# marc345/Dense2Sparse-ViT

Hardware: AMD Instinct MI355X
Metric: training images/s, DeiT-S 224 keep_ratio=0.5 (dense-to-sparse ViT train step, teacher fwd + student fwd/bwd + AdamW) (higher is better)
Workload: dtype f32; 1 GPU; DeiT-Small 224x224 patch16, 1-stage prune keep_ratio=0.5 @ block 3 (196->98 tokens), large LN predictor, kl_div mask loss, per-GPU batch 128; global_batch=128, parallelism=dp1

## Files before the change

dense2sparse-vit_amd/csrc/attention_f32.hip:

```cpp
#include "d2s_common.h"

namespace {

#ifdef D2S_ATTN_STAMPS
__device__ unsigned long long g_attn_stamps[16 * 8192];
#define ASTAMP(i) if (threadIdx.x == 0) { const int L_ = blockIdx.y * gridDim.x + blockIdx.x; if (L_ < 8192) g_attn_stamps[16 * L_ + (i)] = __builtin_amdgcn_s_memtime(); }
#define ASTAMPR(i) if (threadIdx.x == 0) { const int L_ = blockIdx.y * gridDim.x + blockIdx.x; if (L_ < 8192) g_attn_stamps[16 * L_ + (i)] = __builtin_amdgcn_s_memrealtime(); }
#else
#define ASTAMP(i)
#define ASTAMPR(i)
#endif

constexpr int DH = 64;
constexpr int PITCH = 68;

__device__ __forceinline__ void load_rows_regs(const float* __restrict__ base, long ld, int row, int nrows, int half,
                                               float scale, f32x4 (&r)[8]) {
    if (row < nrows) {
        const float* p = base + (long)row * ld + 4 * half;
#pragma unroll
        for (int t = 0; t < 8; ++t) {
            r[t] = *reinterpret_cast<const f32x4*>(p + 8 * t);
#pragma unroll
            for (int j = 0; j < 4; ++j) r[t][j] *= scale;
        }
    } else {
#pragma unroll
        for (int t = 0; t < 8; ++t) r[t] = f32x4{0.f, 0.f, 0.f, 0.f};
    }
}

__device__ __forceinline__ void tile_load(const float* __restrict__ base, long ld, int row0, int nrows, int tid, f32x4 (&r)[2]) {
#pragma unroll
    for (int i = 0; i < 2; ++i) {
        const int f = tid + i * 256, row = row0 + (f >> 4), d4 = (f & 15) * 4;
        r[i] = row < nrows ? *reinterpret_cast<const f32x4*>(base + (long)row * ld + d4) : f32x4{0.f, 0.f, 0.f, 0.f};
    }
}
__device__ __forceinline__ void tile_store(float* __restrict__ S, int tid, const f32x4 (&r)[2]) {
#pragma unroll
    for (int i = 0; i < 2; ++i) {
        const int f = tid + i * 256;
        *reinterpret_cast<f32x4*>(&S[(f >> 4) * PITCH + (f & 15) * 4]) = r[i];
    }
}

__device__ __forceinline__ void mma_lds_reg(const float* __restrict__ S, int l31, int half, const f32x4 (&y)[8], f32x16& acc) {
#pragma unroll
    for (int t = 0; t < 8; ++t) {
        const f32x4 a = *reinterpret_cast<const f32x4*>(&S[l31 * PITCH + 8 * t + 4 * half]);
#pragma unroll
        for (int j = 0; j < 4; ++j) acc = mfma32(a[j], y[t][j], acc);
    }
}
__device__ __forceinline__ void mma_reg_lds(const f32x16& p, const float* __restrict__ S, int l31, int half, f32x16 (&o)[2],
                                            int groups = 4) {
#pragma unroll
    for (int g = 0; g < 4; ++g) {
        if (g < groups) {
#pragma unroll
            for (int r = 4 * g; r < 4 * g + 4; ++r) {
                const float* row = &S[mfma32_row(r, half) * PITCH];
                o[0] = mfma32(p[r], row[l31], o[0]);
                o[1] = mfma32(p[r], row[32 + l31], o[1]);
            }
        }
    }
}

__device__ __forceinline__ void mma_lds_reg_t(const f32x16& p, const float* __restrict__ S, int l31, int half, f32x16 (&o)[2],
                                              int groups = 4) {
#pragma unroll
    for (int g = 0; g < 4; ++g) {
        if (g < groups) {
#pragma unroll
            for (int r = 4 * g; r < 4 * g + 4; ++r) {
                const float* row = &S[mfma32_row(r, half) * PITCH];
                o[0] = mfma32(row[l31], p[r], o[0]);
                o[1] = mfma32(row[32 + l31], p[r], o[1]);
            }
        }
    }
}

struct AttnFwdArgs {
    const float* qkv; float* out; float* lse; float* cls_row;
    const float* policy; float* cinv; const int* cu;
    int n, H; float scale, eps; int total;
};

template <bool POLICY, bool VARLEN, bool KEYW = false>
__global__ __launch_bounds__(256, 3) void attn_fwd_kernel(AttnFwdArgs a) {
    __shared__ __attribute__((aligned(16))) float Ks[32 * PITCH];
    __shared__ __attribute__((aligned(16))) float Vs[32 * PITCH];
    __shared__ float pol_s[32];
    __shared__ __attribute__((aligned(16))) float vred[POLICY ? 16 * 64 : 4];
    __shared__ float vsum_s[64];
    extern __shared__ __attribute__((aligned(16))) float cls_s[];
    const int tid = threadIdx.x, lane = tid & 63, wave = tid >> 6, half = lane >> 5, l31 = lane & 31;
    const int H = a.H;
    ASTAMP(0); ASTAMPR(8);
    int bx, by;
    xcd_remap_2d(bx, by);
    const int b = by / H, h = by % H;
    const long ld = 3L * H * DH;
    const int row_base = VARLEN ? a.cu[b] : 0;
    const int n = VARLEN ? a.cu[b + 1] - row_base : a.n;
    if (VARLEN && bx * 128 >= n) return;
    const long tok0 = VARLEN ? (long)row_base : (long)b * n;
    const float* qb = a.qkv + tok0 * ld + h * DH;
    const float* kb = qb + (long)H * DH;
    const float* vb = kb + (long)H * DH;
    const float* polb = (POLICY || KEYW) ? a.policy + (long)b * n : nullptr;
    const float scale = a.scale;
    const int q0 = bx * 128 + wave * 32;
    const bool active = q0 < n;
    const bool want_cls = a.cls_row != nullptr && bx == 0 && wave == 0;
    const int qi = q0 + l31;

    f32x4 qreg[8];
    load_rows_regs(qb, ld, qi, n, half, scale, qreg);

    f32x16 o[2];
#pragma unroll
    for (int r = 0; r < 16; ++r) { o[0][r] = 0.f; o[1][r] = 0.f; }
    float m_run = -INFINITY, l_run = 0.f;
    f32x4 vacc = {0.f, 0.f, 0.f, 0.f};

    const int ntiles = (n + 31) / 32;
    f32x4 kr[2], vr[2];
    float pr = 0.f;
    tile_load(kb, ld, 0, n, tid, kr);
    tile_load(vb, ld, 0, n, tid, vr);
    if ((POLICY || KEYW) && tid < 32) pr = tid < n ? polb[tid] : 0.f;
    for (int t = 0; t < ntiles; ++t) {
        __syncthreads();
        tile_store(Ks, tid, kr);
        tile_store(Vs, tid, vr);
        if (KEYW && tid < 32) pol_s[tid] = pr;
        if (POLICY) {
            if (tid < 32) pol_s[tid] = pr;
            vacc += vr[0];
            vacc += vr[1];
        }
        __syncthreads();
        if (t == 0) { ASTAMP(1); }
        if (t == 1) { ASTAMP(2); }
        if (t == 2) { ASTAMP(3); }
        if (t + 1 < ntiles) {
            tile_load(kb, ld, (t + 1) * 32, n, tid, kr);
            tile_load(vb, ld, (t + 1) * 32, n, tid, vr);
            if ((POLICY || KEYW) && tid < 32) { const int kj = (t + 1) * 32 + tid; pr = kj < n ? polb[kj] : 0.f; }
        }
        if (!active) continue;
        f32x16 s;
#pragma unroll
        for (int r = 0; r < 16; ++r) s[r] = 0.f;
        mma_lds_reg(Ks, l31, half, qreg, s);
        const int kv0 = t * 32;
        float mt = -INFINITY;
#pragma unroll
        for (int r = 0; r < 16; ++r) {
            if (kv0 + mfma32_row(r, half) >= n) s[r] = -INFINITY;
            mt = fmaxf(mt, s[r]);
        }
        if (want_cls && l31 == 0) {
#pragma unroll
            for (int r = 0; r < 16; ++r) {
                const int key = kv0 + mfma32_row(r, half);
                if (key < n) cls_s[key] = s[r];
            }
        }
        mt = fmaxf(mt, __shfl_xor(mt, 32, 64));
        const float m_new = fmaxf(m_run, mt);
        const float alpha = __expf(m_run - m_new);
        float rs = 0.f;
#pragma unroll
        for (int r = 0; r < 16; ++r) {
            s[r] = __expf(s[r] - m_new);
            if (POLICY) {
                const int kr_ = mfma32_row(r, half);
                s[r] *= (kv0 + kr_ == qi) ? 1.f : pol_s[kr_];
            }
            if (KEYW) s[r] *= pol_s[mfma32_row(r, half)];
            rs += s[r];
        }
        rs += __shfl_xor(rs, 32, 64);
        l_run = l_run * alpha + rs;
        m_run = m_new;
#pragma unroll
        for (int r = 0; r < 16; ++r) {
            o[0][r] *= alpha;
            o[1][r] *= alpha;
        }
        mma_lds_reg_t(s, Vs, l31, half, o, min(4, (n - kv0 + 7) >> 3));
    }
    ASTAMP(4);
    const float c = POLICY ? a.eps / (float)n : 0.f;
    if (POLICY) {
        *reinterpret_cast<f32x4*>(&vred[(tid >> 4) * 64 + (tid & 15) * 4]) = vacc;
        __syncthreads();
        if (tid < 64) {
            float t = 0.f;
#pragma unroll
            for (int g = 0; g < 16; ++g) t += vred[g * 64 + tid];
            vsum_s[tid] = t * c;
        }
        __syncthreads();
    }
    if (!active) return;
    const float inv_l = 1.0f / (POLICY ? l_run + a.eps : l_run);
    if (qi < n) {
        float* p = a.out + (tok0 + qi) * H * DH + h * DH;
#pragma unroll
        for (int dt = 0; dt < 2; ++dt)
#pragma unroll
            for (int g = 0; g < 4; ++g) {
                f32x4 v;
#pragma unroll
                for (int j = 0; j < 4; ++j) {
                    float num = o[dt][4 * g + j];
                    if (POLICY) num += vsum_s[32 * dt + 8 * g + 4 * half + j];
                    v[j] = num * inv_l;
                }
                *reinterpret_cast<f32x4*>(p + 32 * dt + 8 * g + 4 * half) = v;
            }
    }
    const long stat0 = VARLEN ? (long)h * a.total + row_base : ((long)b * H + h) * n;
    if (half == 0 && qi < n) {
        if (a.lse) a.lse[stat0 + qi] = m_run + logf(POLICY ? l_run + a.eps : l_run);
        if (POLICY && a.cinv) a.cinv[stat0 + qi] = c * inv_l;
    }
    if (want_cls) {
        const float m0 = __shfl(m_run, 0, 64), il0 = __shfl(inv_l, 0, 64);
        float* cr = a.cls_row + stat0;
        for (int j = lane; j < n; j += 64) {
            float e = expf(cls_s[j] - m0);
            if (POLICY) e = e * (j == 0 ? 1.f : polb[j]) + c;
            cr[j] = e * il0;
        }
    }
    ASTAMP(5); ASTAMPR(9);
}

__global__ __launch_bounds__(256) void attn_delta_kernel(const float* __restrict__ out, const float* __restrict__ dout,
                                                         float* __restrict__ delta, long rows, int n, int H) {
    const int lane = threadIdx.x & 63;
    const long row = (long)blockIdx.x * 4 + (threadIdx.x >> 6);
    if (row >= rows) return;
    const long b = row / n, i = row - b * n;
    for (int h = 0; h < H; ++h) {
        const long e = row * H * DH + h * DH + lane;
        const float s = wave_sum(out[e] * dout[e]);
        if (lane == 0) delta[(b * H + h) * n + i] = s;
    }
}

__device__ __forceinline__ void tile_load_u32(const float* __restrict__ base, unsigned ld, int row0, int nrows, int tid, f32x4 (&r)[2]) {
#pragma unroll
    for (int i = 0; i < 2; ++i) {
        const int f = tid + i * 256, row = row0 + (f >> 4);
        const unsigned off = (unsigned)row * ld + (unsigned)((f & 15) * 4);
        r[i] = row < nrows ? *reinterpret_cast<const f32x4*>(base + off) : f32x4{0.f, 0.f, 0.f, 0.f};
    }
}

struct VarlenSeg { const int* cu; int total; };
__device__ __forceinline__ int varlen_rows(VarlenSeg v, int b, int max_n, int& row_base) {
    const int r0 = min(max(v.cu[b], 0), v.total), r1 = min(max(v.cu[b + 1], r0), v.total);
    row_base = r0;
    return min(r1 - r0, max_n);
}

template <bool POLICY, bool KEYW = false, bool VARLEN = false>
__global__ __launch_bounds__(256, 3) void attn_bwd_dq_kernel(const float* __restrict__ qkv, const float* __restrict__ dout,
                                                          const float* __restrict__ lse, const float* __restrict__ delta,
                                                          float* __restrict__ dqkv, int n, int H, float scale,
                                                          const float* __restrict__ policy, VarlenSeg varlen) {
    static_assert(!(KEYW && POLICY), "key weights travel in the policy's argument");
    static_assert(!(VARLEN && (POLICY || KEYW)), "the ragged form has neither a policy nor key weights");
    __shared__ __attribute__((aligned(16))) float Ks[32 * PITCH];
    __shared__ __attribute__((aligned(16))) float Vs[32 * PITCH];
    __shared__ float pol_s[32];
    const int tid = threadIdx.x, lane = tid & 63, wave = tid >> 6, half = lane >> 5, l31 = lane & 31;
    int bx, by;
    xcd_remap_2d(bx, by);
    const int b = by / H, h = by % H;
    const long ld = 3L * H * DH, ldo = (long)H * DH;
    int row_base = 0;
    if constexpr (VARLEN) {
        n = varlen_rows(varlen, b, n, row_base);
        if (bx * 128 >= n) return;
    }
    const long stat0v = VARLEN ? (long)h * varlen.total + row_base : 0;
    const float* qb = qkv + (VARLEN ? (long)row_base : (long)b * n) * ld + h * DH;
    const float* kb = qb + (long)H * DH;
    const float* vb = kb + (long)H * DH;
    const float* dob = dout + (VARLEN ? (long)row_base : (long)b * n) * ldo + h * DH;
    const int q0 = bx * 128 + wave * 32;
    const bool active = q0 < n;

    f32x4 qreg[8], doreg[8];
    load_rows_regs(qb, ld, q0 + l31, n, half, scale, qreg);
    load_rows_regs(dob, ldo, q0 + l31, n, half, 1.0f, doreg);
    const bool qok = q0 + l31 < n;
    const float lse_i = qok ? lse[(VARLEN ? stat0v : ((long)b * H + h) * n) + q0 + l31] : INFINITY;
    const float dl_i = qok ? delta[(VARLEN ? stat0v : ((long)b * H + h) * n) + q0 + l31] : 0.f;

    f32x16 dq[2];
#pragma unroll
    for (int r = 0; r < 16; ++r) { dq[0][r] = 0.f; dq[1][r] = 0.f; }

    const int ntiles = (n + 31) / 32;
    f32x4 kr[2], vr[2];
    float pr = 0.f;
    const float* polb = (POLICY || KEYW) ? policy + (long)b * n : nullptr;
    if (VARLEN) {
        tile_load_u32(kb, (unsigned)ld, 0, n, tid, kr);
        tile_load_u32(vb, (unsigned)ld, 0, n, tid, vr);
    } else {
        tile_load(kb, ld, 0, n, tid, kr);
        tile_load(vb, ld, 0, n, tid, vr);
    }
    if ((POLICY || KEYW) && tid < 32) pr = tid < n ? polb[tid] : 0.f;
    for (int t = 0; t < ntiles; ++t) {
        __syncthreads();
        tile_store(Ks, tid, kr);
        tile_store(Vs, tid, vr);
        if ((POLICY || KEYW) && tid < 32) pol_s[tid] = pr;
        __syncthreads();
        if (t + 1 < ntiles) {
            if (VARLEN) {
                tile_load_u32(kb, (unsigned)ld, (t + 1) * 32, n, tid, kr);
                tile_load_u32(vb, (unsigned)ld, (t + 1) * 32, n, tid, vr);
            } else {
                tile_load(kb, ld, (t + 1) * 32, n, tid, kr);
                tile_load(vb, ld, (t + 1) * 32, n, tid, vr);
            }
            if ((POLICY || KEYW) && tid < 32) { const int kj = (t + 1) * 32 + tid; pr = kj < n ? polb[kj] : 0.f; }
        }
        if (!active) continue;
        f32x16 s, dp;
#pragma unroll
        for (int r = 0; r < 16; ++r) { s[r] = 0.f; dp[r] = 0.f; }
        mma_lds_reg(Ks, l31, half, qreg, s);
        mma_lds_reg(Vs, l31, half, doreg, dp);
        const int kv0 = t * 32;
#pragma unroll
        for (int r = 0; r < 16; ++r) {
            const int kr_ = mfma32_row(r, half);
            float p = (kv0 + kr_ < n) ? __expf(s[r] - lse_i) : 0.f;
            if (POLICY) p *= (kv0 + kr_ == q0 + l31) ? 1.f : pol_s[kr_];
            if (KEYW) p *= pol_s[kr_];
            s[r] = p * (dp[r] - dl_i);
        }
        mma_reg_lds(s, Ks, l31, half, dq, min(4, (n - kv0 + 7) >> 3));
    }
    if (!active) return;
    float* dqb = dqkv + (VARLEN ? (long)row_base : (long)b * n) * ld + h * DH;
#pragma unroll
    for (int r = 0; r < 16; ++r) {
        const int qi = q0 + mfma32_row(r, half);
        if (qi < n) {
            float* p = dqb + (long)qi * ld;
            p[l31] = dq[0][r] * scale;
            p[32 + l31] = dq[1][r] * scale;
        }
    }
}

__device__ __forceinline__ void dkv_fetch_next(const float* __restrict__ qb, const float* __restrict__ dob, const float* __restrict__ lse_b,
                                               const float* __restrict__ dl_b, const float* __restrict__ ci_b, unsigned ld, unsigned ldo,
                                               int t1, int n, int tid, f32x4 (&qr)[2], f32x4 (&dr)[2], float& lr, float& dlr, float& cir) {
    tile_load_u32(qb, ld, t1 * 32, n, tid, qr);
    tile_load_u32(dob, ldo, t1 * 32, n, tid, dr);
    if (tid < 32) {
        const unsigned qi = (unsigned)(t1 * 32 + tid);
        lr = qi < (unsigned)n ? lse_b[qi] : INFINITY;
        dlr = qi < (unsigned)n ? dl_b[qi] : 0.f;
        cir = qi < (unsigned)n ? ci_b[qi] : 0.f;
    }
}

template <bool POLICY, bool DPOL = false, bool KEYW = false, bool VARLEN = false>
__global__ __launch_bounds__(256, 2) void attn_bwd_dkv_kernel(const float* __restrict__ qkv, const float* __restrict__ dout,
                                                           const float* __restrict__ lse, const float* __restrict__ delta,
                                                           float* __restrict__ dqkv, int n, int H, float scale,
                                                           const float* __restrict__ policy, const float* __restrict__ cinv,
                                                           float* dpol_part, VarlenSeg varlen) {
    static_assert(!DPOL || POLICY, "the policy's gradient needs a policy");
    static_assert(!(KEYW && POLICY), "key weights travel in the policy's argument");
    static_assert(!(VARLEN && (POLICY || DPOL || KEYW)), "the ragged form has neither a policy nor key weights");
    __shared__ __attribute__((aligned(16))) float Qs[32 * PITCH];
    __shared__ __attribute__((aligned(16))) float Ds[32 * PITCH];
    __shared__ float lse_s[32], dl_s[32], ci_s[32];
    const int tid = threadIdx.x, lane = tid & 63, wave = tid >> 6, half = lane >> 5, l31 = lane & 31;
    int bx, by;
    xcd_remap_2d(bx, by);
    const int b = by / H, h = by % H;
    const long ld = 3L * H * DH, ldo = (long)H * DH;
    int row_base = 0;
    if constexpr (VARLEN) {
        n = varlen_rows(varlen, b, n, row_base);
        if (bx * 128 >= n) return;
    }
    const long tok0 = VARLEN ? (long)row_base : (long)b * n;
    const long stat0 = VARLEN ? (long)h * varlen.total + row_base : ((long)b * H + h) * n;
    const float* qb = qkv + tok0 * ld + h * DH;
    const float* kb = qb + (long)H * DH;
    const float* vb = kb + (long)H * DH;
    const float* dob = dout + tok0 * ldo + h * DH;
    const float* lse_b = lse + stat0;
    const float* dl_b = delta + stat0;
    const int k0 = bx * 128 + wave * 32;
    const bool active = k0 < n;

    f32x4 kreg[8], vreg[8];
    load_rows_regs(kb, ld, k0 + l31, n, half, scale, kreg);
    load_rows_regs(vb, ld, k0 + l31, n, half, 1.0f, vreg);

    f32x16 dk[2], dv[2];
#pragma unroll
    for (int r = 0; r < 16; ++r) { dk[0][r] = 0.f; dk[1][r] = 0.f; dv[0][r] = 0.f; dv[1][r] = 0.f; }

    const int ntiles = (n + 31) / 32;
    f32x4 qr[2], dr[2];
    float lr = 0.f, dlr = 0.f, cir = 0.f;
    float dpol_acc = 0.f;
    const float* ci_b = POLICY ? cinv + ((long)b * H + h) * n : nullptr;
    const float pol_key = ((POLICY || KEYW) && k0 + l31 < n) ? policy[(long)b * n + k0 + l31] : 0.f;
    tile_load(qb, ld, 0, n, tid, qr);
    tile_load(dob, ldo, 0, n, tid, dr);
    if (tid < 32) { lr = tid < n ? lse_b[tid] : INFINITY; dlr = tid < n ? dl_b[tid] : 0.f; if (POLICY) cir = tid < n ? ci_b[tid] : 0.f; }
    for (int t = 0; t < ntiles; ++t) {
        __syncthreads();
        tile_store(Qs, tid, qr);
        tile_store(Ds, tid, dr);
        if (tid < 32) { lse_s[tid] = lr; dl_s[tid] = dlr; if (POLICY) ci_s[tid] = cir; }
        __syncthreads();
        if (!DPOL && t + 1 < ntiles) {
            tile_load(qb, ld, (t + 1) * 32, n, tid, qr);
            tile_load(dob, ldo, (t + 1) * 32, n, tid, dr);
            if (tid < 32) {
                const int qi = (t + 1) * 32 + tid;
                lr = qi < n ? lse_b[qi] : INFINITY;
                dlr = qi < n ? dl_b[qi] : 0.f;
                if (POLICY) cir = qi < n ? ci_b[qi] : 0.f;
            }
        }
        if (DPOL && !active && t + 1 < ntiles) dkv_fetch_next(qb, dob, lse_b, dl_b, ci_b, (unsigned)ld, (unsigned)ldo, t + 1, n, tid, qr, dr, lr, dlr, cir);
        if (!active) continue;
        f32x16 s, dp;
#pragma unroll
        for (int r = 0; r < 16; ++r) { s[r] = 0.f; dp[r] = 0.f; }
        mma_lds_reg(Qs, l31, half, kreg, s);
        mma_lds_reg(Ds, l31, half, vreg, dp);
#pragma unroll
        for (int r = 0; r < 16; ++r) {
            const int qi = mfma32_row(r, half);
            float p = __expf(s[r] - lse_s[qi]);
            if (DPOL) {
                const bool diag = t * 32 + qi == k0 + l31;
                const float g = dp[r] - dl_s[qi];
                dpol_acc += diag ? 0.f : p * g;
                p *= diag ? 1.f : pol_key;
                s[r] = p + ci_s[qi];
                dp[r] = p * g;
                continue;
            }
            if (POLICY) p *= (t * 32 + qi == k0 + l31) ? 1.f : pol_key;
            if (KEYW) p *= pol_key;
            s[r] = POLICY ? p + ci_s[qi] : p;
            dp[r] = p * (dp[r] - dl_s[qi]);
        }
        const int qgroups = min(4, (n - t * 32 + 7) >> 3);
        mma_reg_lds(s, Ds, l31, half, dv, qgroups);
        mma_reg_lds(dp, Qs, l31, half, dk, qgroups);
        if (DPOL && t + 1 < ntiles) dkv_fetch_next(qb, dob, lse_b, dl_b, ci_b, (unsigned)ld, (unsigned)ldo, t + 1, n, tid, qr, dr, lr, dlr, cir);
    }
    if (!active) return;
    int l31e = l31, halfe = half, k0e = k0;
    if constexpr (DPOL) {
        int t2 = (int)threadIdx.x;
        asm volatile("" : "+v"(t2));
        l31e = t2 & 31; halfe = (t2 >> 5) & 1; k0e = bx * 128 + (t2 >> 6) * 32;
        dpol_acc += __shfl_xor(dpol_acc, 32, 64);
        if (halfe == 0 && k0e + l31e < n) dpol_part[((long)b * H + h) * n + k0e + l31e] = dpol_acc;
    }
    float* dkb = dqkv + tok0 * ld + (long)H * DH + h * DH;
    float* dvb = dkb + (long)H * DH;
#pragma unroll
    for (int r = 0; r < 16; ++r) {
        const int ki = k0e + mfma32_row(r, halfe);
        if (ki < n) {
            float* pk = dkb + (long)ki * ld;
            float* pv = dvb + (long)ki * ld;
            pk[l31e] = dk[0][r] * scale;
            pk[32 + l31e] = dk[1][r] * scale;
            pv[l31e] = dv[0][r];
            pv[32 + l31e] = dv[1][r];
        }
    }
}

__global__ __launch_bounds__(256) void attn_dpol_fold_kernel(const float* __restrict__ part, float* __restrict__ dpolicy, int B, int n, int H) {
    const long i = (long)blockIdx.x * 256 + threadIdx.x;
    if (i >= (long)B * n) return;
    const long b = i / n, j = i - b * n;
    float s = 0.f;
    if (j > 0)
        for (int h = 0; h < H; ++h) s += part[(b * H + h) * n + j];
    dpolicy[i] = s;
}

}

#ifdef D2S_ATTN_STAMPS
extern "C" int d2s_debug_read_attn_stamps(unsigned long long* host_out, int n_wg) {
    return hipMemcpyFromSymbol(host_out, HIP_SYMBOL(g_attn_stamps), (size_t)n_wg * 16 * sizeof(unsigned long long)) == hipSuccess ? 0 : -1;
}
#endif

template <bool POLICY, bool VARLEN, bool KEYW = false>
static int attn_fwd_launch(const AttnFwdArgs& a, int B, int n_max, hipStream_t stream) {
    hipLaunchKernelGGL((attn_fwd_kernel<POLICY, VARLEN, KEYW>), dim3((n_max + 127) / 128, B * a.H), dim3(256),
                       a.cls_row ? (size_t)n_max * sizeof(float) : 0, stream, a);
    return d2s_check_launch();
}

template <bool POLICY, bool DPOL = false, bool KEYW = false, bool VARLEN = false>
static int attn_bwd_launch(const float* qkv, const float* out, const float* dout, const float* lse, float* dqkv, float* delta_ws, int B, int n,
                           int H, float scale, hipStream_t stream, const float* policy = nullptr, const float* cinv = nullptr,
                           float* dpolicy = nullptr, float* dpol_ws = nullptr, VarlenSeg seg = VarlenSeg{nullptr, 0}) {
    const long rows = VARLEN ? (long)seg.total : (long)B * n;
    hipLaunchKernelGGL(attn_delta_kernel, dim3((unsigned)((rows + 3) / 4)), dim3(256), 0, stream, out, dout, delta_ws, rows,
                       VARLEN ? seg.total : n, H);
    dim3 grid((n + 127) / 128, B * H), block(256);
    hipLaunchKernelGGL((attn_bwd_dq_kernel<POLICY, KEYW, VARLEN>), grid, block, 0, stream, qkv, dout, lse, delta_ws, dqkv, n, H, scale, policy, seg);
    hipLaunchKernelGGL((attn_bwd_dkv_kernel<POLICY, DPOL, KEYW, VARLEN>), grid, block, 0, stream, qkv, dout, lse, delta_ws, dqkv, n, H, scale,
                       policy, cinv, dpol_ws, seg);
    if (DPOL)
        hipLaunchKernelGGL(attn_dpol_fold_kernel, dim3((unsigned)((rows + 255) / 256)), dim3(256), 0, stream, dpol_ws, dpolicy, B, n, H);
    return d2s_check_launch();
}

static int attn_varlen_fwd(const float* qkv, const int* cu_seqlens, float* out, float* lse, float* cls_row, int B, int total, int max_n, int H,
                           float scale, hipStream_t stream) {
    if (!qkv || !cu_seqlens || !out || B <= 0 || total <= 0 || max_n <= 0 || max_n > 8192 || H <= 0) return D2S_ERR_ARG;
    return attn_fwd_launch<false, true>(AttnFwdArgs{qkv, out, lse, cls_row, nullptr, nullptr, cu_seqlens, 0, H, scale, 0.f, total}, B, max_n, stream);
}

extern "C" {

int d2s_attn_fwd_f32(const float* qkv, float* out, float* lse, float* cls_row, int B, int n, int H, float scale,
                     hipStream_t stream) {
    if (!qkv || !out || !lse || B <= 0 || n <= 0 || H <= 0 || n > 8192) return D2S_ERR_ARG;
    return attn_fwd_launch<false, false>(AttnFwdArgs{qkv, out, lse, cls_row, nullptr, nullptr, nullptr, n, H, scale, 0.f, 0}, B, n, stream);
}

int d2s_attn_policy_fwd_f32(const float* qkv, const float* policy, float* out, float* lse, float* cinv, float* cls_row, int B, int n,
                            int H, float scale, float eps, hipStream_t stream) {
    if (!qkv || !policy || !out || !lse || !cinv || B <= 0 || n <= 0 || H <= 0 || n > 8192) return D2S_ERR_ARG;
    return attn_fwd_launch<true, false>(AttnFwdArgs{qkv, out, lse, cls_row, policy, cinv, nullptr, n, H, scale, eps, 0}, B, n, stream);
}

int d2s_attn_varlen_fwd_f32(const float* qkv, const int* cu_seqlens, float* out, float* cls_row, int B, int total, int max_n, int H,
                            float scale, hipStream_t stream) {
    return attn_varlen_fwd(qkv, cu_seqlens, out, nullptr, cls_row, B, total, max_n, H, scale, stream);
}

int d2s_attn_varlen_fwd_lse_f32(const float* qkv, const int* cu_seqlens, float* out, float* lse, float* cls_row, int B, int total, int max_n,
                                int H, float scale, hipStream_t stream) {
    if (!lse) return D2S_ERR_ARG;
    return attn_varlen_fwd(qkv, cu_seqlens, out, lse, cls_row, B, total, max_n, H, scale, stream);
}

int d2s_attn_varlen_bwd_f32(const float* qkv, const int* cu_seqlens, const float* out, const float* dout, const float* lse, float* dqkv,
                            float* delta_ws, int B, int total, int max_n, int H, float scale, hipStream_t stream) {
    if (!qkv || !cu_seqlens || !out || !dout || !lse || !dqkv || !delta_ws || B <= 0 || total <= 0 || max_n <= 0 || max_n > 8192 || H <= 0)
        return D2S_ERR_ARG;
    if ((long)max_n * 3 * H * 64 >= (1L << 32)) return D2S_ERR_ARG;
    return attn_bwd_launch<false, false, false, true>(qkv, out, dout, lse, dqkv, delta_ws, B, max_n, H, scale, stream, nullptr, nullptr, nullptr,
                                                      nullptr, VarlenSeg{cu_seqlens, total});
}

int d2s_attn_keyw_fwd_f32(const float* qkv, const float* key_w, float* out, float* lse, int B, int n, int H, float scale, hipStream_t stream) {
    if (!qkv || !key_w || !out || B <= 0 || n < 2 || H <= 0 || n > 8192) return D2S_ERR_ARG;
    return attn_fwd_launch<false, false, true>(AttnFwdArgs{qkv, out, lse, nullptr, key_w, nullptr, nullptr, n, H, scale, 0.f, 0}, B, n, stream);
}

int d2s_attn_delta(const float* out, const float* dout, float* delta, int B, int n, int H, hipStream_t stream) {
    if (!out || !dout || !delta || B <= 0 || n <= 0 || H <= 0) return D2S_ERR_ARG;
    const long rows = (long)B * n;
    hipLaunchKernelGGL(attn_delta_kernel, dim3((unsigned)((rows + 3) / 4)), dim3(256), 0, stream, out, dout, delta, rows, n, H);
    return d2s_check_launch();
}

int d2s_attn_bwd_f32(const float* qkv, const float* out, const float* dout, const float* lse, float* dqkv, float* delta_ws, int B,
                     int n, int H, float scale, hipStream_t stream) {
    if (!qkv || !out || !dout || !lse || !dqkv || !delta_ws || B <= 0 || n <= 0 || H <= 0) return D2S_ERR_ARG;
    return attn_bwd_launch<false>(qkv, out, dout, lse, dqkv, delta_ws, B, n, H, scale, stream);
}

int d2s_attn_keyw_bwd_f32(const float* qkv, const float* key_w, const float* out, const float* dout, const float* lse, float* dqkv,
                          float* delta_ws, int B, int n, int H, float scale, hipStream_t stream) {
    if (!qkv || !key_w || !out || !dout || !lse || !dqkv || !delta_ws || B <= 0 || n < 2 || H <= 0 || n > 8192) return D2S_ERR_ARG;
    return attn_bwd_launch<false, false, true>(qkv, out, dout, lse, dqkv, delta_ws, B, n, H, scale, stream, key_w);
}

int d2s_attn_policy_bwd_f32(const float* qkv, const float* policy, const float* out, const float* dout, const float* lse,
                            const float* cinv, float* dqkv, float* delta_ws, int B, int n, int H, float scale, hipStream_t stream) {
    if (!qkv || !policy || !out || !dout || !lse || !cinv || !dqkv || !delta_ws || B <= 0 || n <= 0 || H <= 0) return D2S_ERR_ARG;
    return attn_bwd_launch<true>(qkv, out, dout, lse, dqkv, delta_ws, B, n, H, scale, stream, policy, cinv);
}

int d2s_attn_policy_bwd_dpol_f32(const float* qkv, const float* policy, const float* out, const float* dout, const float* lse,
                                 const float* cinv, float* dqkv, float* delta_ws, float* dpolicy, float* dpol_ws, int B, int n, int H,
                                 float scale, hipStream_t stream) {
    if (!qkv || !policy || !out || !dout || !lse || !cinv || !dqkv || !delta_ws || !dpolicy || !dpol_ws || B <= 0 || n <= 0 || H <= 0)
        return D2S_ERR_ARG;
    if ((long)n * 3 * H * 64 >= (1L << 32)) return D2S_ERR_ARG;
    return attn_bwd_launch<true, true>(qkv, out, dout, lse, dqkv, delta_ws, B, n, H, scale, stream, policy, cinv, dpolicy, dpol_ws);
}

}
```

Baseline: 3616 images/s.

## Handle small remainder key/query tiles with scalar FMA instead of full MFMA tiles

When the sequence length leaves a final tile of at most eight rows (e.g. n=197 or 99 with cls token), the attention forward, dq and dkv kernels now process that last tile with cross-half-wave dot products and scalar FMAs instead of a full 32-row MFMA tile. This is meant to avoid wasting most of an MFMA tile on padding rows. It adds permlane swaps, an LDS transpose buffer for the backward kernels and extra code paths, which may raise register and LDS pressure and affect occupancy.

```diff
diff --git a/dense2sparse-vit_amd/csrc/attention_f32.hip b/dense2sparse-vit_amd/csrc/attention_f32.hip
--- a/dense2sparse-vit_amd/csrc/attention_f32.hip
+++ b/dense2sparse-vit_amd/csrc/attention_f32.hip
@@ -78,6 +78,87 @@
                 const float* row = &S[mfma32_row(r, half) * PITCH];
                 o[0] = mfma32(row[l31], p[r], o[0]);
                 o[1] = mfma32(row[32 + l31], p[r], o[1]);
+            }
+        }
+    }
+}
+
+__device__ __forceinline__ int remainder_rows(int n) { const int rem = n & 31; return rem <= 8 ? rem : 0; }
+__device__ __forceinline__ int remainder_row_at(int i) { return (i >> 1) + 4 * (i & 1); }
+
+__device__ __forceinline__ void half_wave_pair_of(float a, float b, float& x, float& y) {
+    const auto sw = __builtin_amdgcn_permlane32_swap(__float_as_uint(a), __float_as_uint(b), false, false);
+    x = __uint_as_float(sw[0]);
+    y = __uint_as_float(sw[1]);
+}
+__device__ __forceinline__ void dot_rows_lds_reg(const float* __restrict__ S, int half, const f32x4 (&y)[8], int rem, f32x4& s4) {
+    float c[4] = {0.f, 0.f, 0.f, 0.f};
+    const int ni = (rem + 1) >> 1;
+    const float* X = S + half * PITCH;
+#pragma unroll
+    for (int t = 0; t < 8; ++t) {
+        float ylo[4], yhi[4];
+#pragma unroll
+        for (int j = 0; j < 4; ++j) half_wave_pair_of(y[t][j], y[t][j], ylo[j], yhi[j]);
+#pragma unroll
+        for (int i = 0; i < 4; ++i) {
+            if (i < ni) {
+                const f32x4 alo = *reinterpret_cast<const f32x4*>(&X[2 * i * PITCH + 8 * t]);
+                const f32x4 ahi = *reinterpret_cast<const f32x4*>(&X[2 * i * PITCH + 8 * t + 4]);
+#pragma unroll
+                for (int j = 0; j < 4; ++j) {
+                    c[i] = __builtin_fmaf(alo[j], ylo[j], c[i]);
+                    c[i] = __builtin_fmaf(ahi[j], yhi[j], c[i]);
+                }
+            }
+        }
+    }
+    float r0, r1, r2, r3;
+    half_wave_pair_of(c[0], c[2], r0, r1);
+    half_wave_pair_of(c[1], c[3], r2, r3);
+    s4 = f32x4{r0, r1, r2, r3};
+}
+__device__ __forceinline__ float remainder_row_value(const f32x4& p4, int k, int half) {
+    float v = p4[0];
+#pragma unroll
+    for (int r = 1; r < 4; ++r) v = (k & 3) == r ? p4[r] : v;
+    const float other = __shfl_xor(v, 32, 64);
+    return (k >> 2) == half ? v : other;
+}
+__device__ __forceinline__ void fma_lds_reg_t(const f32x4& p4, const float* __restrict__ S, int half, int rem, f32x16 (&o)[2]) {
+#pragma unroll 1
+    for (int i = 0; i < 8; ++i) {
+        const int k = remainder_row_at(i);
+        if (k >= rem) continue;
+        const float pk = remainder_row_value(p4, k, half);
+#pragma unroll
+        for (int dt = 0; dt < 2; ++dt)
+#pragma unroll
+            for (int g = 0; g < 4; ++g) {
+                const f32x4 v = *reinterpret_cast<const f32x4*>(&S[k * PITCH + 32 * dt + 8 * g + 4 * half]);
+#pragma unroll
+                for (int j = 0; j < 4; ++j) o[dt][4 * g + j] = __builtin_fmaf(v[j], pk, o[dt][4 * g + j]);
+            }
+    }
+}
+__device__ __forceinline__ void fma_reg_lds(const f32x4& p4, const float* __restrict__ S, float* T, int l31, int half, int rem,
+                                            f32x16 (&o)[2]) {
+    __builtin_amdgcn_wave_barrier();
+#pragma unroll
+    for (int r = 0; r < 4; ++r) T[(4 * half + r) * 32 + l31] = p4[r];
+    __builtin_amdgcn_wave_barrier();
+#pragma unroll 1
+    for (int i = 0; i < 8; ++i) {
+        const int k = remainder_row_at(i);
+        if (k >= rem) continue;
+        const float s0 = S[k * PITCH + l31], s1 = S[k * PITCH + 32 + l31];
+#pragma unroll
+        for (int g = 0; g < 4; ++g) {
+            const f32x4 w = *reinterpret_cast<const f32x4*>(&T[k * 32 + 8 * g + 4 * half]);
+#pragma unroll
+            for (int j = 0; j < 4; ++j) {
+                o[0][4 * g + j] = __builtin_fmaf(w[j], s0, o[0][4 * g + j]);
+                o[1][4 * g + j] = __builtin_fmaf(w[j], s1, o[1][4 * g + j]);
             }
         }
     }
@@ -128,12 +209,51 @@
     f32x4 vacc = {0.f, 0.f, 0.f, 0.f};
 
     const int ntiles = (n + 31) / 32;
+    const int rem_last = remainder_rows(n), ntiles_mma = ntiles - (rem_last ? 1 : 0);
     f32x4 kr[2], vr[2];
     float pr = 0.f;
     tile_load(kb, ld, 0, n, tid, kr);
     tile_load(vb, ld, 0, n, tid, vr);
     if ((POLICY || KEYW) && tid < 32) pr = tid < n ? polb[tid] : 0.f;
-    for (int t = 0; t < ntiles; ++t) {
+    auto softmax_step = [&](auto& s, int kv0, auto nr) {
+        constexpr int NR = decltype(nr)::value;
+        float mt = -INFINITY;
+#pragma unroll
+        for (int r = 0; r < NR; ++r) {
+            if (kv0 + mfma32_row(r, half) >= n) s[r] = -INFINITY;
+            mt = fmaxf(mt, s[r]);
+        }
+        if (want_cls && l31 == 0) {
+#pragma unroll
+            for (int r = 0; r < NR; ++r) {
+                const int key = kv0 + mfma32_row(r, half);
+                if (key < n) cls_s[key] = s[r];
+            }
+        }
+        mt = fmaxf(mt, __shfl_xor(mt, 32, 64));
+        const float m_new = fmaxf(m_run, mt);
+        const float alpha = __expf(m_run - m_new);
+        float rs = 0.f;
+#pragma unroll
+        for (int r = 0; r < NR; ++r) {
+            s[r] = __expf(s[r] - m_new);
+            if (POLICY) {
+                const int kr_ = mfma32_row(r, half);
+                s[r] *= (kv0 + kr_ == qi) ? 1.f : pol_s[kr_];
+            }
+            if (KEYW) s[r] *= pol_s[mfma32_row(r, half)];
+            rs += s[r];
+        }
+        rs += __shfl_xor(rs, 32, 64);
+        l_run = l_run * alpha + rs;
+        m_run = m_new;
+#pragma unroll
+        for (int r = 0; r < 16; ++r) {
+            o[0][r] *= alpha;
+            o[1][r] *= alpha;
+        }
+    };
+    auto stage_tile = [&]() {
         __syncthreads();
         tile_store(Ks, tid, kr);
         tile_store(Vs, tid, vr);
@@ -144,6 +264,9 @@
             vacc += vr[1];
         }
         __syncthreads();
+    };
+    for (int t = 0; t < ntiles_mma; ++t) {
+        stage_tile();
         if (t == 0) { ASTAMP(1); }
         if (t == 1) { ASTAMP(2); }
         if (t == 2) { ASTAMP(3); }
@@ -153,47 +276,22 @@
             if ((POLICY || KEYW) && tid < 32) { const int kj = (t + 1) * 32 + tid; pr = kj < n ? polb[kj] : 0.f; }
         }
         if (!active) continue;
+        const int kv0 = t * 32;
         f32x16 s;
 #pragma unroll
         for (int r = 0; r < 16; ++r) s[r] = 0.f;
         mma_lds_reg(Ks, l31, half, qreg, s);
-        const int kv0 = t * 32;
-        float mt = -INFINITY;
-#pragma unroll
-        for (int r = 0; r < 16; ++r) {
-            if (kv0 + mfma32_row(r, half) >= n) s[r] = -INFINITY;
-            mt = fmaxf(mt, s[r]);
-        }
-        if (want_cls && l31 == 0) {
-#pragma unroll
-            for (int r = 0; r < 16; ++r) {
-                const int key = kv0 + mfma32_row(r, half);
-                if (key < n) cls_s[key] = s[r];
-            }
-        }
-        mt = fmaxf(mt, __shfl_xor(mt, 32, 64));
-        const float m_new = fmaxf(m_run, mt);
-        const float alpha = __expf(m_run - m_new);
-        float rs = 0.f;
-#pragma unroll
-        for (int r = 0; r < 16; ++r) {
-            s[r] = __expf(s[r] - m_new);
-            if (POLICY) {
-                const int kr_ = mfma32_row(r, half);
-                s[r] *= (kv0 + kr_ == qi) ? 1.f : pol_s[kr_];
-            }
-            if (KEYW) s[r] *= pol_s[mfma32_row(r, half)];
-            rs += s[r];
-        }
-        rs += __shfl_xor(rs, 32, 64);
-        l_run = l_run * alpha + rs;
-        m_run = m_new;
-#pragma unroll
-        for (int r = 0; r < 16; ++r) {
-            o[0][r] *= alpha;
-            o[1][r] *= alpha;
-        }
+        softmax_step(s, kv0, std::integral_constant<int, 16>{});
         mma_lds_reg_t(s, Vs, l31, half, o, min(4, (n - kv0 + 7) >> 3));
+    }
+    if (rem_last) {
+        stage_tile();
+        if (active) {
+            f32x4 s4;
+            dot_rows_lds_reg(Ks, half, qreg, rem_last, s4);
+            softmax_step(s4, (ntiles - 1) * 32, std::integral_constant<int, 4>{});
+            fma_lds_reg_t(s4, Vs, half, rem_last, o);
+        }
     }
     ASTAMP(4);
     const float c = POLICY ? a.eps / (float)n : 0.f;
@@ -282,6 +380,7 @@
     __shared__ __attribute__((aligned(16))) float Ks[32 * PITCH];
     __shared__ __attribute__((aligned(16))) float Vs[32 * PITCH];
     __shared__ float pol_s[32];
+    __shared__ __attribute__((aligned(16))) float tr_s[4 * 8 * 32];
     const int tid = threadIdx.x, lane = tid & 63, wave = tid >> 6, half = lane >> 5, l31 = lane & 31;
     int bx, by;
     xcd_remap_2d(bx, by);
@@ -304,6 +403,7 @@
     load_rows_regs(qb, ld, q0 + l31, n, half, scale, qreg);
     load_rows_regs(dob, ldo, q0 + l31, n, half, 1.0f, doreg);
     const bool qok = q0 + l31 < n;
+    const int wave_u = __builtin_amdgcn_readfirstlane(wave);
     const float lse_i = qok ? lse[(VARLEN ? stat0v : ((long)b * H + h) * n) + q0 + l31] : INFINITY;
     const float dl_i = qok ? delta[(VARLEN ? stat0v : ((long)b * H + h) * n) + q0 + l31] : 0.f;
 
@@ -312,6 +412,7 @@
     for (int r = 0; r < 16; ++r) { dq[0][r] = 0.f; dq[1][r] = 0.f; }
 
     const int ntiles = (n + 31) / 32;
+    const int rem_last = remainder_rows(n), ntiles_mma = ntiles - (rem_last ? 1 : 0);
     f32x4 kr[2], vr[2];
     float pr = 0.f;
     const float* polb = (POLICY || KEYW) ? policy + (long)b * n : nullptr;
@@ -323,12 +424,26 @@
         tile_load(vb, ld, 0, n, tid, vr);
     }
     if ((POLICY || KEYW) && tid < 32) pr = tid < n ? polb[tid] : 0.f;
-    for (int t = 0; t < ntiles; ++t) {
+    auto ds_step = [&](auto& s, const auto& dp, int kv0, int half, auto nr) {
+        constexpr int NR = decltype(nr)::value;
+#pragma unroll
+        for (int r = 0; r < NR; ++r) {
+            const int kr_ = mfma32_row(r, half);
+            float p = (kv0 + kr_ < n) ? __expf(s[r] - lse_i) : 0.f;
+            if (POLICY) p *= (kv0 + kr_ == q0 + l31) ? 1.f : pol_s[kr_];
+            if (KEYW) p *= pol_s[kr_];
+            s[r] = p * (dp[r] - dl_i);
+        }
+    };
+    auto stage_tile = [&]() {
         __syncthreads();
         tile_store(Ks, tid, kr);
         tile_store(Vs, tid, vr);
         if ((POLICY || KEYW) && tid < 32) pol_s[tid] = pr;
         __syncthreads();
+    };
+    for (int t = 0; t < ntiles_mma; ++t) {
+        stage_tile();
         if (t + 1 < ntiles) {
             if (VARLEN) {
                 tile_load_u32(kb, (unsigned)ld, (t + 1) * 32, n, tid, kr);
@@ -340,31 +455,37 @@
             if ((POLICY || KEYW) && tid < 32) { const int kj = (t + 1) * 32 + tid; pr = kj < n ? polb[kj] : 0.f; }
         }
         if (!active) continue;
+        const int kv0 = t * 32;
         f32x16 s, dp;
 #pragma unroll
         for (int r = 0; r < 16; ++r) { s[r] = 0.f; dp[r] = 0.f; }
         mma_lds_reg(Ks, l31, half, qreg, s);
         mma_lds_reg(Vs, l31, half, doreg, dp);
-        const int kv0 = t * 32;
-#pragma unroll
-        for (int r = 0; r < 16; ++r) {
-            const int kr_ = mfma32_row(r, half);
-            float p = (kv0 + kr_ < n) ? __expf(s[r] - lse_i) : 0.f;
-            if (POLICY) p *= (kv0 + kr_ == q0 + l31) ? 1.f : pol_s[kr_];
-            if (KEYW) p *= pol_s[kr_];
-            s[r] = p * (dp[r] - dl_i);
-        }
+        ds_step(s, dp, kv0, half, std::integral_constant<int, 16>{});
         mma_reg_lds(s, Ks, l31, half, dq, min(4, (n - kv0 + 7) >> 3));
+    }
+    int lane_r = (int)__builtin_amdgcn_mbcnt_hi(~0u, __builtin_amdgcn_mbcnt_lo(~0u, 0u));
+    asm volatile("" : "+v"(lane_r));
+    const int half_r = lane_r >> 5, l31_r = lane_r & 31, q0_r = bx * 128 + wave_u * 32;
+    if (rem_last) {
+        stage_tile();
+        if (active) {
+            f32x4 s4, dp4;
+            dot_rows_lds_reg(Ks, half_r, qreg, rem_last, s4);
+            dot_rows_lds_reg(Vs, half_r, doreg, rem_last, dp4);
+            ds_step(s4, dp4, (ntiles - 1) * 32, half_r, std::integral_constant<int, 4>{});
+            fma_reg_lds(s4, Ks, &tr_s[wave_u * 256], l31_r, half_r, rem_last, dq);
+        }
     }
     if (!active) return;
     float* dqb = dqkv + (VARLEN ? (long)row_base : (long)b * n) * ld + h * DH;
 #pragma unroll
     for (int r = 0; r < 16; ++r) {
-        const int qi = q0 + mfma32_row(r, half);
+        const int qi = q0_r + mfma32_row(r, half_r);
         if (qi < n) {
             float* p = dqb + (long)qi * ld;
-            p[l31] = dq[0][r] * scale;
-            p[32 + l31] = dq[1][r] * scale;
+            p[l31_r] = dq[0][r] * scale;
+            p[32 + l31_r] = dq[1][r] * scale;
         }
     }
 }
@@ -394,6 +515,7 @@
     __shared__ __attribute__((aligned(16))) float Qs[32 * PITCH];
     __shared__ __attribute__((aligned(16))) float Ds[32 * PITCH];
     __shared__ float lse_s[32], dl_s[32], ci_s[32];
+    __shared__ __attribute__((aligned(16))) float tr_s[4 * 8 * 32];
     const int tid = threadIdx.x, lane = tid & 63, wave = tid >> 6, half = lane >> 5, l31 = lane & 31;
     int bx, by;
     xcd_remap_2d(bx, by);
@@ -414,6 +536,7 @@
     const float* dl_b = delta + stat0;
     const int k0 = bx * 128 + wave * 32;
     const bool active = k0 < n;
+    const int wave_u = __builtin_amdgcn_readfirstlane(wave);
 
     f32x4 kreg[8], vreg[8];
     load_rows_regs(kb, ld, k0 + l31, n, half, scale, kreg);
@@ -424,6 +547,7 @@
     for (int r = 0; r < 16; ++r) { dk[0][r] = 0.f; dk[1][r] = 0.f; dv[0][r] = 0.f; dv[1][r] = 0.f; }
 
     const int ntiles = (n + 31) / 32;
+    const int rem_last = remainder_rows(n), ntiles_mma = ntiles - (rem_last ? 1 : 0);
     f32x4 qr[2], dr[2];
     float lr = 0.f, dlr = 0.f, cir = 0.f;
     float dpol_acc = 0.f;
@@ -432,12 +556,36 @@
     tile_load(qb, ld, 0, n, tid, qr);
     tile_load(dob, ldo, 0, n, tid, dr);
     if (tid < 32) { lr = tid < n ? lse_b[tid] : INFINITY; dlr = tid < n ? dl_b[tid] : 0.f; if (POLICY) cir = tid < n ? ci_b[tid] : 0.f; }
-    for (int t = 0; t < ntiles; ++t) {
+    auto stage_tile = [&]() {
         __syncthreads();
         tile_store(Qs, tid, qr);
         tile_store(Ds, tid, dr);
         if (tid < 32) { lse_s[tid] = lr; dl_s[tid] = dlr; if (POLICY) ci_s[tid] = cir; }
         __syncthreads();
+    };
+    auto pds_step = [&](auto& s, auto& dp, int t, int half, int key, auto nr) {
+        constexpr int NR = decltype(nr)::value;
+#pragma unroll
+        for (int r = 0; r < NR; ++r) {
+            const int qi = mfma32_row(r, half);
+            float p = __expf(s[r] - lse_s[qi]);
+            if (DPOL) {
+                const bool diag = t * 32 + qi == key;
+                const float g = dp[r] - dl_s[qi];
+                dpol_acc += diag ? 0.f : p * g;
+                p *= diag ? 1.f : pol_key;
+                s[r] = p + ci_s[qi];
+                dp[r] = p * g;
+            } else {
+                if (POLICY) p *= (t * 32 + qi == key) ? 1.f : pol_key;
+                if (KEYW) p *= pol_key;
+                s[r] = POLICY ? p + ci_s[qi] : p;
+                dp[r] = p * (dp[r] - dl_s[qi]);
+            }
+        }
+    };
+    for (int t = 0; t < ntiles_mma; ++t) {
+        stage_tile();
         if (!DPOL && t + 1 < ntiles) {
             tile_load(qb, ld, (t + 1) * 32, n, tid, qr);
             tile_load(dob, ldo, (t + 1) * 32, n, tid, dr);
@@ -455,35 +603,28 @@
         for (int r = 0; r < 16; ++r) { s[r] = 0.f; dp[r] = 0.f; }
         mma_lds_reg(Qs, l31, half, kreg, s);
         mma_lds_reg(Ds, l31, half, vreg, dp);
-#pragma unroll
-        for (int r = 0; r < 16; ++r) {
-            const int qi = mfma32_row(r, half);
-            float p = __expf(s[r] - lse_s[qi]);
-            if (DPOL) {
-                const bool diag = t * 32 + qi == k0 + l31;
-                const float g = dp[r] - dl_s[qi];
-                dpol_acc += diag ? 0.f : p * g;
-                p *= diag ? 1.f : pol_key;
-                s[r] = p + ci_s[qi];
-                dp[r] = p * g;
-                continue;
-            }
-            if (POLICY) p *= (t * 32 + qi == k0 + l31) ? 1.f : pol_key;
-            if (KEYW) p *= pol_key;
-            s[r] = POLICY ? p + ci_s[qi] : p;
-            dp[r] = p * (dp[r] - dl_s[qi]);
-        }
+        pds_step(s, dp, t, half, k0 + l31, std::integral_constant<int, 16>{});
         const int qgroups = min(4, (n - t * 32 + 7) >> 3);
         mma_reg_lds(s, Ds, l31, half, dv, qgroups);
         mma_reg_lds(dp, Qs, l31, half, dk, qgroups);
         if (DPOL && t + 1 < ntiles) dkv_fetch_next(qb, dob, lse_b, dl_b, ci_b, (unsigned)ld, (unsigned)ldo, t + 1, n, tid, qr, dr, lr, dlr, cir);
     }
+    int lane_e = (int)__builtin_amdgcn_mbcnt_hi(~0u, __builtin_amdgcn_mbcnt_lo(~0u, 0u));
+    asm volatile("" : "+v"(lane_e));
+    const int l31e = lane_e & 31, halfe = lane_e >> 5, k0e = bx * 128 + wave_u * 32;
+    if (rem_last) {
+        stage_tile();
+        if (active) {
+            f32x4 s4, dp4;
+            dot_rows_lds_reg(Qs, halfe, kreg, rem_last, s4);
+            dot_rows_lds_reg(Ds, halfe, vreg, rem_last, dp4);
+            pds_step(s4, dp4, ntiles - 1, halfe, k0e + l31e, std::integral_constant<int, 4>{});
+            fma_reg_lds(s4, Ds, &tr_s[wave_u * 256], l31e, halfe, rem_last, dv);
+            fma_reg_lds(dp4, Qs, &tr_s[wave_u * 256], l31e, halfe, rem_last, dk);
+        }
+    }
     if (!active) return;
-    int l31e = l31, halfe = half, k0e = k0;
     if constexpr (DPOL) {
-        int t2 = (int)threadIdx.x;
-        asm volatile("" : "+v"(t2));
-        l31e = t2 & 31; halfe = (t2 >> 5) & 1; k0e = bx * 128 + (t2 >> 6) * 32;
         dpol_acc += __shfl_xor(dpol_acc, 32, 64);
         if (halfe == 0 && k0e + l31e < n) dpol_part[((long)b * H + h) * n + k0e + l31e] = dpol_acc;
     }
```

Result: no change. 3599 images/s (-0.5%).
